# quang-ha/lammps-sph-multiphase

Measured on AMD Instinct MI355X. Metric: particle-steps/s + achieved HBM GB/s, 1M-particle taitwater+rhosum, 1/2/4/8 GPUs, higher is better.
Workload: dtype f64

## Files before the change

### include/sph_hip.h

```cpp
#ifndef SPH_HIP_H
#define SPH_HIP_H

#include <stdint.h>

#ifdef __cplusplus
extern "C" {
#endif

#define SPH_HIP_ABI_VERSION 2

#define SPH_HIP_OK 0
#define SPH_HIP_EINVAL (-1)
#define SPH_HIP_ENODEV (-2)
#define SPH_HIP_ERUNTIME (-3)
#define SPH_HIP_ENOMEM (-4)
#define SPH_HIP_ECOMM (-5)
#define SPH_HIP_EOVERFLOW (-6)

#define SPH_LIST_FULL 0
#define SPH_LIST_HALF 1

#define SPH_VISC_MONAGHAN 0
#define SPH_VISC_MORRIS 1

// ... 124 lines not shown
  int rank;
  int sort;
  int kernel_path;
  const sph_engine_mp_config *mp;
} sph_engine_config;

typedef struct {
  int64_t step;
  int nlocal, nghost;
  int64_t nbr_full;
  int nbr_builds;
  int nbr_maxrow;
  int staged;
  int stage_max;
  double ms_rhosum, ms_tait, ms_heat, ms_integrate, ms_comm, ms_neigh;
  int64_t n_rhosum, n_tait, n_heat, n_neigh;
  int blk_nbig;
  int inner_rows;
  int inner_live;
  int flags;
  int64_t inner_refresh;
} sph_engine_stats;

#define SPH_STAT_RHO_FUSED (1 << 0)
#define SPH_STAT_BLK_R32 (1 << 1)
#define SPH_STAT_BLK_BIGIMG (1 << 2)
#define SPH_STAT_BLK_NOPRE (1 << 3)
#define SPH_STAT_BLK_ROWRETRY (1 << 4)
#define SPH_STAT_BLK_IMGRETRY (1 << 5)
#define SPH_STAT_MP_W4 (1 << 6)
#define SPH_STAT_MP_POW (1 << 7)
#define SPH_STAT_MP_ROW (1 << 8)
#define SPH_STAT_MP_RHO_LISTFILL (1 << 9)

typedef struct sph_engine sph_engine;

int sph_engine_create(int device, const sph_engine_config *cfg, sph_engine **out);
int sph_engine_destroy(sph_engine *e);

int sph_engine_comm_uid(void *uid128);
int sph_engine_comm_init(sph_engine *e, const void *uid128, int nranks, int rank);
int sph_engine_comm_loopback(sph_engine *e, int on);
typedef struct sph_local_world sph_local_world;
int sph_local_world_create(int nranks, sph_local_world **out);
int sph_local_world_destroy(sph_local_world *w);
int sph_engine_comm_local(sph_engine *e, sph_local_world *w, int rank);
int sph_engine_comm_ipc(sph_engine *e, const char *name, int nranks, int rank, int mode);
#define SPH_TUNE_OVERLAP 1
#define SPH_TUNE_BLKUMF 2
int sph_engine_tune(sph_engine *e, int key, int value);
int sph_engine_set_tags(sph_engine *e, const int *tags);

int sph_engine_set_atoms(sph_engine *e, int n, const double *x, const double *v,
                         const int *type, const double *rho, const double *en,
                         const double *cv);
int sph_engine_set_atoms_multiphase(sph_engine *e, const double *rmass, const double *cv,
                                    const double *cg);
int sph_engine_phase_change(sph_engine *e, const sph_phasechange_params *p, int nevery,
                            int seed);
int sph_engine_atom_sort(sph_engine *e, int sortfreq, double binsize);

#define SPH_REGION_SPHERE 0
#define SPH_REGION_BLOCK 1
typedef struct {
  int style;
  int interior;
  double xc, yc, zc, radius;
  double xlo, xhi, ylo, yhi, zlo, zhi;
} sph_region;

#define SPH_MAX_SETMESO 8
#define SPH_SET_RHO 0
#define SPH_SET_E 1
#define SPH_SET_T 2
#define SPH_SET_DE 3
typedef struct {
  int what;
  double value;
  int type_mask;
  int region_mode;
  sph_region region;
} sph_setmeso;
int sph_engine_setmeso(sph_engine *e, const sph_setmeso *fix);
// ... 44 lines not shown
```

### lammps-sph-multiphase_amd/__init__.py

```python
from __future__ import annotations

import ctypes as C
import os

import numpy as np

HERE = os.path.dirname(os.path.abspath(__file__))
LIB_PATH = os.environ.get("SPH_HIP_LIB") or os.path.join(HERE, "libsph_hip.so")
HEADER = os.path.join(os.path.dirname(HERE), "include", "sph_hip.h")

SPH_LIST_FULL, SPH_LIST_HALF = 0, 1
SPH_VISC_MONAGHAN, SPH_VISC_MORRIS = 0, 1
SPH_MAXTYPES = 8
_NT2 = (SPH_MAXTYPES + 1) ** 2

ERRORS = {-1: "EINVAL", -2: "ENODEV", -3: "ERUNTIME", -4: "ENOMEM", -5: "ECOMM",
          -6: "EOVERFLOW"}


class HipError(RuntimeError):
    def __init__(self, code: int, msg: str):
        super().__init__(f"sph_hip {ERRORS.get(code, code)}: {msg}")
        self.code = code

# ... 151 lines not shown
    "sph_hip_host_arrays": (_i, [_vp, _i, _vp, _vp, _vp, _vp, _vp, _vp, _vp]),
    "sph_hip_list_csr": (_i, [_vp, _i, _i, _lp, _ip]),
    "sph_hip_build_list": (_i, [_vp, _i, C.c_int64, _dp]),
    "sph_hip_list_numneigh": (_i, [_vp, _ip]),
    "sph_hip_rhosum": (_i, [_vp, _dp]),
    "sph_hip_taitwater": (_i, [_vp, _dp, _dp, _dp, _vp]),
    "sph_hip_heatconduction": (_i, [_vp, _dp]),
    "sph_hip_atoms_multiphase": (_i, [_vp, _dp, _vp]),
    "sph_hip_rhosum_multiphase_coeff": (_i, [_vp, _dp]),
    "sph_hip_rhosum_multiphase": (_i, [_vp, _dp]),
    "sph_hip_taitwater_multiphase_coeff": (_i, [_vp, _dp, _dp, _dp, _dp, _dp, _dp]),
    "sph_hip_taitwater_multiphase": (_i, [_vp, _dp]),
    "sph_hip_heatconduction_phasechange_coeff": (_i, [_vp, _dp, _vp, _vp, _dp]),
    "sph_hip_heatconduction_phasechange": (_i, [_vp, _dp]),
    "sph_hip_colorgradient_coeff": (_i, [_vp, _dp, _dp]),
    "sph_hip_colorgradient": (_i, [_vp, _dp]),
    "sph_hip_set_timing": (_i, [_vp, _i]),
    "sph_hip_last_kernel_ms": (_i, [_vp, _dp]),
    "sph_hip_surfacetension_coeff": (_i, [_vp, _dp]),
    "sph_hip_surfacetension": (_i, [_vp, _dp, _dp]),
    "sph_hip_phasechange": (_i, [_vp, _vp, C.POINTER(_i), _dp, _dp, _dp, _dp, _i,
                                 C.POINTER(_i), _vp, _vp]),
    "sph_hip_phasechange_finish": (_i, [_i, _dp, _dp, _dp]),
    "sph_engine_create": (_i, [_i, C.POINTER(EngineConfig), C.POINTER(_vp)]),
    "sph_engine_destroy": (_i, [_vp]),
    "sph_engine_comm_uid": (_i, [_vp]),
    "sph_engine_comm_init": (_i, [_vp, _vp, _i, _i]),
    "sph_engine_comm_loopback": (_i, [_vp, _i]),
    "sph_local_world_create": (_i, [_i, C.POINTER(_vp)]),
    "sph_local_world_destroy": (_i, [_vp]),
    "sph_engine_comm_local": (_i, [_vp, _vp, _i]),
    "sph_engine_comm_ipc": (_i, [_vp, C.c_char_p, _i, _i, _i]),
    "sph_engine_tune": (_i, [_vp, _i, _i]),
    "sph_engine_set_tags": (_i, [_vp, _ip]),
    "sph_engine_set_atoms": (_i, [_vp, _i, _dp, _dp, _ip, _dp, _vp, _vp]),
    "sph_engine_setup": (_i, [_vp]),
    "sph_engine_run": (_i, [_vp, _i]),
    "sph_engine_nlocal": (_i, [_vp]),
    "sph_engine_get_atoms": (_i, [_vp, _vp, _vp, _vp, _vp, _vp, _vp, _vp, _vp]),
    "sph_engine_neighbor_counts": (_i, [_vp, _ip]),
    "sph_engine_stats_get": (_i, [_vp, C.POINTER(EngineStats)]),
    "sph_engine_set_timing": (_i, [_vp, _i]),
    "sph_engine_sync": (_i, [_vp]),
    "sph_engine_pair_passes": (_i, [_vp, _i]),
    "sph_engine_rebuild_passes": (_i, [_vp, _i]),
    "sph_engine_set_atoms_multiphase": (_i, [_vp, _dp, _vp, _vp]),
    "sph_engine_phase_change": (_i, [_vp, _vp, _i, _i]),
    "sph_engine_atom_sort": (_i, [_vp, _i, C.c_double]),
    "sph_engine_get_atoms_multiphase": (_i, [_vp, _vp, _vp, _vp, _vp, _vp, _vp]),
    "sph_engine_write_restart": (_i, [_vp, _vp, C.c_int64, C.POINTER(_i)]),
    "sph_engine_read_restart": (_i, [_vp, _i, _dp]),
}


def load() -> C.CDLL:
    global _lib
    if _lib is None:
        if not os.path.exists(LIB_PATH):
            raise HipError(-2, f"{LIB_PATH} not built (run `make -C lammps-sph-multiphase_amd`)")
        L = C.CDLL(LIB_PATH)
        for name, (res, args) in EXPORTS.items():
            fn = getattr(L, name)
            fn.restype = res
            fn.argtypes = args
        _lib = L
    return _lib
# ... 444 lines not shown
            for c in classes:
                mask |= 1 << c
            _chk(self.L.sph_engine_set_timing(self.h, mask << 1))
        else:
            _chk(self.L.sph_engine_set_timing(self.h, 1 if on else 0))

    @property
    def nlocal(self):
        return self.L.sph_engine_nlocal(self.h)

    def get_atoms(self):
        n = self.nlocal
        out = {k: np.zeros((n, 3)) for k in ("x", "v", "f")}
        out.update({k: np.zeros(n) for k in ("rho", "e", "drho", "de")})
        out["tag"] = np.zeros(n, dtype=np.int32)
        _chk(self.L.sph_engine_get_atoms(self.h, out["x"].ctypes.data, out["v"].ctypes.data,
                                         out["rho"].ctypes.data, out["e"].ctypes.data,
                                         out["f"].ctypes.data, out["drho"].ctypes.data,
                                         out["de"].ctypes.data, out["tag"].ctypes.data))
        return out

    def set_tags(self, tags):
        tags = np.ascontiguousarray(tags, dtype=np.int32)
        _chk(self.L.sph_engine_set_tags(self.h, tags))

    def comm_local(self, world: "LocalWorld", rank: int):
        _chk(self.L.sph_engine_comm_local(self.h, world.h, rank))
        self._world = world

    def comm_init(self, uid: bytes, nranks: int, rank: int):
        buf = C.create_string_buffer(bytes(uid), 128)
        _chk(self.L.sph_engine_comm_init(self.h, buf, nranks, rank))

    TUNE_OVERLAP, TUNE_BLKUMF = 1, 2

    def tune(self, key: int, value: int):
        _chk(self.L.sph_engine_tune(self.h, key, int(value)))

    IPC_DEVICE, IPC_HOST = 0, 1

    def comm_ipc(self, name: str, nranks: int, rank: int, mode: int = 0):
        _chk(self.L.sph_engine_comm_ipc(self.h, name.encode(), nranks, rank, int(mode)))

    def comm_loopback(self, on: bool = True):
        _chk(self.L.sph_engine_comm_loopback(self.h, 1 if on else 0))

    def neighbor_counts(self):
        c = np.zeros(self.nlocal, dtype=np.int32)
        _chk(self.L.sph_engine_neighbor_counts(self.h, c))
        return c

    STAT_RHO_FUSED, STAT_BLK_R32, STAT_BLK_BIGIMG = 1 << 0, 1 << 1, 1 << 2
    STAT_BLK_NOPRE, STAT_BLK_ROWRETRY, STAT_BLK_IMGRETRY = 1 << 3, 1 << 4, 1 << 5
    STAT_MP_W4, STAT_MP_POW, STAT_MP_ROW, STAT_MP_RHO_LISTFILL = 1 << 6, 1 << 7, 1 << 8, 1 << 9

    def stats(self) -> dict:
        s = EngineStats()
        _chk(self.L.sph_engine_stats_get(self.h, C.byref(s)))
        return s.as_dict()


def unpack_restart_records(buf):
    buf = np.asarray(buf)
    mp = buf.shape[1] == 21
    ints = (lambda c: buf[:, c].astype(np.int64)) if mp else (lambda c: buf[:, c].view(np.int64))
    img = ints(7)
    d = {"x": buf[:, 1:4], "tag": ints(4), "type": ints(5), "image": img,
         "image_xyz": np.stack([(img & 1023) - 512, ((img >> 10) & 1023) - 512,
                                ((img >> 20) & 1023) - 512], 1)}
    return d


def write_dump_custom(fp, step, atoms, columns, boxlo, boxhi, boundary="pp pp pp"):
    lo, hi = np.asarray(boxlo, float), np.asarray(boxhi, float)
    prd = hi - lo
    n = atoms["x"].shape[0]
    img = atoms.get("image", np.zeros((n, 3), np.int64))
    cols = []
    for c in columns:
        if c == "id":
            cols.append((atoms["tag"] + 1, True))
        elif c == "type":
            cols.append((atoms["type"], True))
        elif c in ("x", "y", "z"):
            cols.append((atoms["x"][:, "xyz".index(c)], False))
        elif c in ("xs", "ys", "zs"):
            k = "xyz".index(c[0])
# ... 26 lines not shown
```

### lammps-sph-multiphase_amd/csrc/sph_engine.hip

```cpp
#include <hip/hip_runtime.h>
#include <hipcub/hipcub.hpp>
#include <rocprofiler-sdk-roctx/roctx.h>

#include <algorithm>
#include <chrono>
#include <cstring>
#include <cmath>
#include <vector>

#include "sph_coef.h"
#include "sph_comm.h"
#include "sph_dispatch.h"
#include "sph_blk_kernels.h"
#include "sph_engine_kernels.h"
#include "sph_engine_mp.h"
#include "sph_fix_kernels.h"
#include "sph_ipc.h"
#include "sph_mp2_kernels.h"
#include "sph_pc.h"
#include "sph_row2_kernels.h"
#include "sph_util.h"

using namespace sph;

// ... 154 lines not shown
  bool global_tags = false;
  int last_build = 0;

  DBuf<double4> xf, vr;
  DBuf<double> en;
  DBuf<int> ty;
  DBuf<double4> vel, fo;
  DBuf<double> de;
  DBuf<int> tag;
  DBuf<double4> xf2, vr2, vel2;
  DBuf<double> en2;
  DBuf<int> ty2, tag2;
  DBuf<int> gowner, gimg;
  DBuf<int> gorank, goidx;
  bool dr_ok = false;
  std::vector<int> dr_peer;
  std::vector<size_t> dr_soff, dr_roff;
  DBuf<int> dr_sidx, dr_rslot, dr_self, dr_req;
  DBuf<int> dr_byq, dr_byg, dr_hist;
  int dr_nself = 0;
  std::vector<const void *> dr_sb;
  std::vector<void *> dr_rb;
  std::vector<size_t> dr_sbytes, dr_rbytes;
  DBuf<unsigned char> flags;
  DBuf<int> sel, nsel;
  Bins bn{};
  int nbins = 0;
  QBins qb{};
  int nqbins = 0;
  DBuf<int> qbeg, tb, xpos;
  DBuf<double4> xb;
  DBuf<unsigned> bkey, bkey2;
  DBuf<int> bidx, bidx2;
  DBuf<int> cnt, off, nbr;
  int64_t nbr_total = 0;
  int nbr_builds = 0, nbr_maxrow = 0;
  int64_t inner_refreshes = 0;
  bool strided = false;
  int list_stride = 0;
  int list_perm_g = 0;
  bool list_tbits = false;
  bool blk = false;
  int blk_sh = 0, blk_um = 0, blk_umf = 0, blk_sstride = 0, blk_rowcap = 0;
  DBuf<int> ulist, ucnt, kcnt;
  DBuf<unsigned short> snbr;
  DBuf<int> uilist, uicnt;
  bool blk_ksmall = false;
  int blk_kover = 0;
  int blk_flags = 0, blk_retry = 0;
  int mp_flags = 0;
  DBuf<unsigned short> snbi;
  DBuf<int> icnt, moved;
  DBuf<double4> x0;
  double inner_margin = 0.0;
  bool inner = false, inner_written = false;
  DBuf<int> nbs;
  DBuf<int> mx, ccnt;
  DBuf<long long> blen;
  DBuf<unsigned char> tmp;
  int *h_scalar = nullptr;
  int *h_small = nullptr;

  bool timing = false;
  int timing_mask = 0;
  struct EvPair {
    hipEvent_t a, b;
// ... 49 lines not shown
    }
    pending.clear();
  }

  void tmp_reserve(size_t b) { tmp.reserve(b); }

  void ensure_atoms(size_t nall, bool keep) {
    xf.reserve(nall, keep, s);
    vr.reserve(nall, keep, s);
    en.reserve(nall, keep, s);
    ty.reserve(nall, keep, s);
    if (mp) {
      vel.reserve(nall, keep, s);
      rm.reserve(nall, keep, s);
      cvv.reserve(nall, keep, s);
      cg.reserve(nall, keep, s);
    }
  }
  void mpx_copy(int n, const int *src, int first, DBuf<double> &buf) {
    if (!mp || n <= 0) return;
    buf.reserve((size_t)MPX * n, false, s);
    hipLaunchKernelGGL(k_mpx_pack, dim3(blocks(n)), dim3(BLK), 0, s, n, src, vel.p, rm.p, cvv.p,
                       cg.p, buf.p);
    hipLaunchKernelGGL(k_mpx_unpack, dim3(blocks(n)), dim3(BLK), 0, s, n, (const int *)nullptr,
                       first, buf.p, vel.p, rm.p, cvv.p, cg.p);
  }
  bool nt1() const { return cfg.ntypes == 1; }
  int blk_visc() const {
    if (nt1() && cfg.tait_visc == SPH_VISC_MONAGHAN && hc.tait[3].viscC == 0.0)
      return BLK_VISC_NONE;
    return cfg.tait_visc;
  }

  void sort_owned() {
    if (nlocal < 1) return;
    const int n = nlocal;
    bkey.reserve(n);
    bkey2.reserve(n);
    bidx.reserve(n);
    bidx2.reserve(n);
    const int div = morton_div();
    Bins kbn = bn;
    for (int k = 0; k < 3; k++)
      if (bn.nb[k] > 1) {
        kbn.nb[k] = bn.nb[k] * div;
        kbn.inv[k] = bn.inv[k] * div;
      }
    if (want_blk()) {
      for (int k = 0; k < 3; k++) {
        const double ext = subhi[k] - sublo[k];
        if (k >= cfg.dim || ext <= 0.0) {
          kbn.lo[k] = sublo[k];
          kbn.nb[k] = 1;
          kbn.inv[k] = 0.0;
          continue;
        }
        const int nc0 = std::max(1, (int)std::ceil(ext / (cutneighmax / div)));
        int nc = 1;
        while (nc < nc0 && nc < 1024) nc *= 2;
        if (!hil_pow2()) nc = std::min(nc0, 1024);
        kbn.lo[k] = sublo[k];
        kbn.nb[k] = nc;
        kbn.inv[k] = nc / ext;
      }
    }
    const bool mort = kbn.nb[0] <= 1024 && kbn.nb[1] <= 1024 && kbn.nb[2] <= 1024;
    if (!mort) kbn = bn;
    int cb = 1;
    const int mx3 = std::max(kbn.nb[0], std::max(kbn.nb[1], kbn.nb[2]));
    while ((1 << cb) < mx3) cb++;
    const bool hil = mort && want_blk() && cb >= 2;
    hipLaunchKernelGGL(k_bin_keys, dim3(blocks(n)), dim3(BLK), 0, s, n, 0, kbn, xf.p, bkey.p,
                       bidx.p, hil ? cb + 1 : (mort ? 1 : 0), cfg.dim);
    int kb = 1;
    if (mort) {
      kb = cb * (hil ? cfg.dim : 3);
    } else {
      while ((1u << kb) < (unsigned)nbins && kb < 32) kb++;
    }
    size_t tb = 0;
    SPH_HIP_TRY(hipcub::DeviceRadixSort::SortPairs(nullptr, tb, bkey.p, bkey2.p, bidx.p, bidx2.p, n, 0, kb, s));
    tmp_reserve(tb);
    SPH_HIP_TRY(hipcub::DeviceRadixSort::SortPairs(tmp.p, tb, bkey.p, bkey2.p, bidx.p, bidx2.p, n, 0, kb, s));
    if (mp) {
      xbuf.reserve((size_t)MPX * n, false, s);
      hipLaunchKernelGGL(k_mpx_pack, dim3(blocks(n)), dim3(BLK), 0, s, n, bidx2.p, vel.p, rm.p,
                         cvv.p, cg.p, xbuf.p);
    }
    grow_twins();
    hipLaunchKernelGGL(k_permute, dim3(blocks(n)), dim3(BLK), 0, s, n, bidx2.p, xf.p, vr.p,
                       en.p, ty.p, vel.p, tag.p, xf2.p, vr2.p, en2.p, ty2.p, vel2.p, tag2.p);
    std::swap(xf, xf2);
    std::swap(vr, vr2);
    std::swap(en, en2);
    std::swap(ty, ty2);
    std::swap(vel, vel2);
    std::swap(tag, tag2);
    if (pc) {
      lidx2.reserve_exact(lidx.cap);
      hipLaunchKernelGGL(k_lidx_take, dim3(blocks(n)), dim3(BLK), 0, s, n, bidx2.p, lidx.p, 0,
                         (const int *)nullptr, lidx2.p);
      std::swap(lidx, lidx2);
    }
    if (mp)
      hipLaunchKernelGGL(k_mpx_unpack, dim3(blocks(n)), dim3(BLK), 0, s, n, (const int *)nullptr,
                         0, xbuf.p, vel.p, rm.p, cvv.p, cg.p);
  }

  void grow_twins() {
    xf2.reserve_exact(xf.cap);
    vr2.reserve_exact(vr.cap);
    en2.reserve_exact(en.cap);
    ty2.reserve_exact(ty.cap);
    vel2.reserve_exact(vel.cap);
    tag2.reserve_exact(tag.cap);
  }
// ... 718 lines not shown
      const double ext = bn.nb[k] > 0 && bn.inv[k] > 0.0 ? bn.nb[k] / bn.inv[k] : 0.0;
      int nb = 1;
      if (k < cfg.dim) {
        nb = (int)(ext / (0.5 * cutneighmax / (k == 0 ? fx : 1)));
        if (nb < 1) nb = 1;
        if (nb > 8192) nb = 8192;
      }
      qb.lo[k] = bn.lo[k];
      qb.nb[k] = nb;
      qb.inv[k] = (k < cfg.dim) ? nb / ext : 0.0;
      qb.size[k] = (k < cfg.dim) ? ext / nb : 1.0;
    }
    qb.cutmaxsq = cutneighmax * cutneighmax;
    nqbins = qb.nb[0] * qb.nb[1] * qb.nb[2];
  }

  void bin_q() {
    const int nall = nlocal + nghost;
    Bins b;
    for (int k = 0; k < 3; k++) {
      b.lo[k] = qb.lo[k];
      b.inv[k] = qb.inv[k];
      b.nb[k] = qb.nb[k];
    }
    bkey.reserve(nall);
    bkey2.reserve(nall);
    bidx.reserve(nall);
    bidx2.reserve(nall);
    qbeg.reserve(nqbins + 1);
    xb.reserve(nall);
    tb.reserve(nall);
    SPH_REQUIRE(!mp || (long long)nall < MP_MAXALL, SPH_HIP_EOVERFLOW,
                "multiphase lists index at most 2^28 atoms per rank (%d)", nall);
    hipLaunchKernelGGL(k_bin_keys, dim3(blocks(nall)), dim3(BLK), 0, s, nall, 0, b, xf.p,
                       bkey.p, bidx.p, 0);
    int endbit = 1;
    while ((1u << endbit) < (unsigned)nqbins && endbit < 32) endbit++;
    size_t tbytes = 0;
    SPH_HIP_TRY(hipcub::DeviceRadixSort::SortPairs(nullptr, tbytes, bkey.p, bkey2.p, bidx.p, bidx2.p, nall, 0, endbit, s));
    tmp_reserve(tbytes);
    SPH_HIP_TRY(hipcub::DeviceRadixSort::SortPairs(tmp.p, tbytes, bkey.p, bkey2.p, bidx.p, bidx2.p, nall, 0, endbit, s));
    hipLaunchKernelGGL(k_lower_bound, dim3(blocks(nqbins + 1)), dim3(BLK), 0, s, nqbins, nall,
                       0, bkey2.p, qbeg.p);
    xpos.reserve(nall);
    hipLaunchKernelGGL(k_bin_copy, dim3(blocks(nall)), dim3(BLK), 0, s, nall, bidx2.p, xf.p,
                       ty.p, xb.p, tb.p, xpos.p, mp ? 1 : 0);
  }
  void list_q(bool csr, const double4 *xi = nullptr) {
    const int n = nlocal, nall = nlocal + nghost;
    const double4 *const xi_src = xi ? xi : xf.p;
    const bool rho = mp && !xi && rhofuse_env() && mpc.rhosum_nstep > 0 &&
                     step % mpc.rhosum_nstep == 0;
    SPH_REQUIRE(!mp || (long long)nall < MP_MAXALL, SPH_HIP_EOVERFLOW,
                "multiphase lists index at most 2^28 atoms per rank (%d)", nall);
    if (rho) rho_tmp.reserve(nlocal + nghost);
    rho_fused_step = rho ? step : -1;
    ccnt.reserve(n + 1);
    off.reserve(n + 1);
    constexpr int G = 8;
    dim3 grid(grid_for_rows(n, G)), block(BLK);
    auto launch = [&](bool fill, int stride, int *dst = nullptr) {
      if (n == 0) return;
      const bool t = nt1();
      const int *const tgp = (mp && !mp2_symmetric(hm)) ? tag.p : (const int *)nullptr;
      int *const cnt_out = (!fill || stride > 0) ? ccnt.p : (int *)nullptr;
      int *const rows = dst ? dst : nbr.p;
// ... 1097 lines not shown
                                                   : cfg->boxlo[k] + e->box.prd[k] * hi;
      auto at = [&](int dx, int dy, int dz) {
        const int l[3] = {(e->myloc[0] + dx + e->pg[0]) % e->pg[0],
                          (e->myloc[1] + dy + e->pg[1]) % e->pg[1],
                          (e->myloc[2] + dz + e->pg[2]) % e->pg[2]};
        return (l[2] * e->pg[1] + l[1]) * e->pg[0] + l[0];
      };
      e->procneigh[k][0] = at(k == 0 ? -1 : 0, k == 1 ? -1 : 0, k == 2 ? -1 : 0);
      e->procneigh[k][1] = at(k == 0 ? 1 : 0, k == 1 ? 1 : 0, k == 2 ? 1 : 0);
      if (e->box.periodic[k])
        SPH_REQUIRE(e->cutghost < e->box.prd[k], SPH_HIP_EINVAL,
                    "ghost cutoff %g >= box length %g in dim %d (multi-hop borders unsupported)",
                    e->cutghost, e->box.prd[k], k);
      if (e->pg[k] > 1)
        SPH_REQUIRE(e->cutghost < e->subhi[k] - e->sublo[k], SPH_HIP_EINVAL,
                    "ghost cutoff %g >= brick width %g in dim %d (multi-hop swaps unsupported)",
                    e->cutghost, e->subhi[k] - e->sublo[k], k);
    }
    e->sc.dtv = cfg->dt;
    e->sc.dtf = 0.5 * cfg->dt * (cfg->ftm2v > 0 ? cfg->ftm2v : 1.0);
    for (int t = 0; t <= nt; t++) e->sc.mass[t] = cfg->mass[t];
    e->sc.stationary_mask = cfg->stationary_mask;
    e->setup_bins_geometry();
    SPH_HIP_TRY(hipStreamCreateWithFlags(&e->s, hipStreamNonBlocking));
    SPH_HIP_TRY(hipMalloc(&e->dc, sizeof(Coefs)));
    SPH_HIP_TRY(hipMemcpy(e->dc, &e->hc, sizeof(Coefs), hipMemcpyHostToDevice));
    if (e->mp) {
      SPH_HIP_TRY(hipMalloc(&e->dm, sizeof(MpCoefs)));
      mp_inverses(e->hm);
      SPH_HIP_TRY(hipMemcpy(e->dm, &e->hm, sizeof(MpCoefs), hipMemcpyHostToDevice));
    }
    SPH_HIP_TRY(hipHostMalloc(&e->h_scalar, sizeof(int)));
    SPH_HIP_TRY(hipHostMalloc(&e->h_small, 16 * sizeof(int)));
  } catch (...) {
    delete e;
    throw;
  }
  e->overlap = false;
  *out = e;
  SPH_API_END
}

int sph_engine_destroy(sph_engine *e) {
  if (!e) return SPH_HIP_OK;
  (void)hipSetDevice(e->device);
  if (e->s) (void)hipStreamSynchronize(e->s);
  if (e->s2) (void)hipStreamSynchronize(e->s2);
  for (auto *b : {&e->xf, &e->vr, &e->vel, &e->fo, &e->xf2, &e->vr2, &e->vel2, &e->xb}) b->release();
  for (auto *b : {&e->en, &e->en2, &e->de, &e->rm, &e->cvv, &e->rho_tmp, &e->dmass, &e->xbuf,
                  &e->xbuf2})
    b->release();
  for (auto *b : {&e->rhoS, &e->rhoF}) b->release();
  for (auto *b : {&e->cg, &e->cgS, &e->cgF, &e->recA, &e->recK, &e->recF, &e->recS}) b->release();
  if (e->dm) (void)hipFree(e->dm);
  for (auto *b : {&e->nbs, &e->gorank, &e->goidx, &e->dr_sidx, &e->dr_rslot, &e->dr_self, &e->dr_req, &e->dr_byq, &e->dr_byg, &e->dr_hist, &e->pc_flag,
                  &e->pc_cand, &e->pc_otag, &e->pc_idx})
    b->release();
  for (auto *b : {&e->pc_rec, &e->pc_gat, &e->pc_Wd, &e->pc_vals, &e->pc_nrec, &e->pc_v0,
                  &e->pc_v1})
    b->release();
  e->pc_k0.release();
  e->pc_k1.release();
  e->pc_cnt.release();
  e->red_part.release();
  e->red_out.release();
  for (auto *b : {&e->ty, &e->ty2, &e->tag, &e->tag2, &e->gowner, &e->gimg, &e->sel, &e->nsel,
                  &e->bidx, &e->bidx2, &e->cnt, &e->off, &e->nbr, &e->mx,
                  &e->ccnt, &e->qbeg, &e->tb, &e->xpos, &e->sel2, &e->rows_in, &e->rows_bd,
                  &e->ulist, &e->ucnt, &e->kcnt, &e->uilist, &e->uicnt})
    b->release();
  for (auto *b : {&e->bkey, &e->bkey2}) b->release();
  for (auto *b : {&e->flags, &e->tmp, &e->cbs, &e->cbr, &e->flag2, &e->fl_in, &e->fl_bd}) b->release();
  e->snbr.release();
  e->snbi.release();
  e->icnt.release();
  e->moved.release();
  e->x0.release();
  e->blen.release();
  for (auto &sw : e->swaps) sw.list.release();
  for (auto &p : e->pending) {
    (void)hipEventDestroy(p.a);
    (void)hipEventDestroy(p.b);
  }
  for (auto ev : e->evpool) (void)hipEventDestroy(ev);
  if (e->h_scalar) (void)hipHostFree(e->h_scalar);
  if (e->h_small) (void)hipHostFree(e->h_small);
  delete e->tr;
  if (e->dc) (void)hipFree(e->dc);
  if (e->ev_fork) (void)hipEventDestroy(e->ev_fork);
  if (e->ev_join) (void)hipEventDestroy(e->ev_join);
  if (e->s2) (void)hipStreamDestroy(e->s2);
  if (e->s) (void)hipStreamDestroy(e->s);
  delete e;
  return SPH_HIP_OK;
}

int sph_engine_set_atoms(sph_engine *e, int n, const double *x, const double *v,
                         const int *type, const double *rho, const double *en,
                         const double *cv) {
  SPH_API_BEGIN
  SPH_REQUIRE(e && n >= 0 && (n == 0 || (x && v && type && rho)), SPH_HIP_EINVAL,
              "sph_engine_set_atoms: bad argument");
  SPH_HIP_TRY(hipSetDevice(e->device));
  for (int i = 0; i < n; i++)
// ... 473 lines not shown
  st->nghost = e->nghost;
  st->nbr_full = e->list_entries();
  st->nbr_builds = e->nbr_builds;
  st->nbr_maxrow = e->nbr_maxrow;
  st->staged = e->blk ? 1 : 0;
  st->stage_max = e->blk ? e->blk_um : 0;
  st->ms_rhosum = e->ms[T_RHO];
  st->ms_tait = e->ms[T_TAIT];
  st->ms_heat = e->ms[T_HEAT];
  st->ms_integrate = e->ms[T_INT];
  st->ms_comm = e->ms[T_COMM];
  st->ms_neigh = e->ms[T_NEIGH];
  st->n_rhosum = e->nlaunch[T_RHO];
  st->n_tait = e->nlaunch[T_TAIT];
  st->n_heat = e->nlaunch[T_HEAT];
  st->n_neigh = e->nlaunch[T_NEIGH];
  st->blk_nbig = 0;
  if (e->blk && e->mx.p) {
    SPH_HIP_TRY(hipMemcpyAsync(&st->blk_nbig, e->mx.p + 9, sizeof(int), hipMemcpyDeviceToHost,
                               e->s));
    SPH_HIP_TRY(hipStreamSynchronize(e->s));
  }
  st->inner_rows = e->inner ? 1 : 0;
  st->inner_live = 0;
  if (e->inner && e->moved.p) {
    int mv = 1;
    SPH_HIP_TRY(hipMemcpyAsync(&mv, e->moved_flag(), sizeof(int), hipMemcpyDeviceToHost, e->s));
    SPH_HIP_TRY(hipStreamSynchronize(e->s));
    st->inner_live = mv == 0 ? 1 : 0;
  }
  st->flags = (e->rho_fused_step >= 0 && e->rho_fused_step == e->step) ? SPH_STAT_RHO_FUSED : 0;
  if (e->blk) st->flags |= e->blk_flags;
  if (e->mp) st->flags |= e->mp_flags;
  st->inner_refresh = e->inner_refreshes;
  SPH_API_END
}

int sph_engine_set_timing(sph_engine *e, int on) {
  SPH_API_BEGIN
  SPH_REQUIRE(e, SPH_HIP_EINVAL, "sph_engine_set_timing: NULL engine");
  SPH_HIP_TRY(hipSetDevice(e->device));
  e->harvest();
  e->timing_mask = on == 1 ? (1 << T_NCLASS) - 1 : (on > 1 ? (on >> 1) & ((1 << T_NCLASS) - 1) : 0);
  e->timing = e->timing_mask != 0;
  for (int k = 0; k < T_NCLASS; k++) {
    e->ms[k] = 0.0;
    e->nlaunch[k] = 0;
  }
  SPH_API_END
}

int sph_engine_sync(sph_engine *e) {
  SPH_API_BEGIN
  SPH_REQUIRE(e, SPH_HIP_EINVAL, "sph_engine_sync: NULL engine");
  SPH_HIP_TRY(hipSetDevice(e->device));
  SPH_HIP_TRY(hipStreamSynchronize(e->s));
  SPH_API_END
}

int sph_engine_comm_uid(void *uid128) {
  SPH_API_BEGIN
  SPH_REQUIRE(uid128, SPH_HIP_EINVAL, "sph_engine_comm_uid: NULL buffer");
  static_assert(sizeof(ncclUniqueId) == 128, "ncclUniqueId is 128 bytes");
  ncclUniqueId id;
  SPH_NCCL_TRY(ncclGetUniqueId(&id));
  memcpy(uid128, &id, sizeof(id));
// ... 41 lines not shown

int sph_local_world_destroy(sph_local_world *w) {
  delete reinterpret_cast<LocalWorld *>(w);
  return SPH_HIP_OK;
}

int sph_engine_comm_local(sph_engine *e, sph_local_world *w, int rank) {
  SPH_API_BEGIN
  SPH_REQUIRE(e && w, SPH_HIP_EINVAL, "sph_engine_comm_local: NULL argument");
  LocalWorld *lw = reinterpret_cast<LocalWorld *>(w);
  SPH_REQUIRE(rank >= 0 && rank < lw->n, SPH_HIP_EINVAL, "rank %d outside [0,%d)", rank, lw->n);
  attach(e, new LocalTransport(lw, rank));
  SPH_API_END
}

int sph_engine_comm_ipc(sph_engine *e, const char *name, int nranks, int rank, int mode) {
  SPH_API_BEGIN
  SPH_REQUIRE(e && name, SPH_HIP_EINVAL, "sph_engine_comm_ipc: NULL argument");
  SPH_HIP_TRY(hipSetDevice(e->device));
  attach(e, new IpcTransport(name, nranks, rank, mode, e->device));
  SPH_API_END
}

int sph_engine_tune(sph_engine *e, int key, int value) {
  SPH_API_BEGIN
  SPH_REQUIRE(e, SPH_HIP_EINVAL, "sph_engine_tune: NULL engine");
  SPH_REQUIRE(!e->setup_done, SPH_HIP_EINVAL, "sph_engine_tune: before sph_engine_setup");
  switch (key) {
    case SPH_TUNE_OVERLAP: e->overlap = value != 0; break;
    case SPH_TUNE_BLKUMF:
      SPH_REQUIRE(value >= 0, SPH_HIP_EINVAL, "sph_engine_tune: BLKUMF %d < 0", value);
      e->blkumf = value;
      break;
    default: SPH_REQUIRE(false, SPH_HIP_EINVAL, "sph_engine_tune: unknown key %d", key);
  }
  SPH_API_END
}

int sph_engine_set_tags(sph_engine *e, const int *tags) {
  SPH_API_BEGIN
  SPH_REQUIRE(e && (tags || e->nlocal == 0), SPH_HIP_EINVAL, "sph_engine_set_tags: bad argument");
  SPH_HIP_TRY(hipSetDevice(e->device));
  int mx = -1;
  for (int i = 0; i < e->nlocal; i++) {
    SPH_REQUIRE(tags[i] >= 0 && tags[i] < (1 << 30), SPH_HIP_EINVAL,
                "sph_engine_set_tags: tag %d outside [0, 2^30)", tags[i]);
    mx = std::max(mx, tags[i]);
  }
  if (e->nlocal)
    SPH_HIP_TRY(hipMemcpy(e->tag.p, tags, e->nlocal * sizeof(int), hipMemcpyHostToDevice));
  e->global_tags = true;
  e->tag_next = mx + 1;
  e->pc_tags_agreed = false;
  e->lidx_valid = false;
  SPH_API_END
}

int sph_engine_atom_sort(sph_engine *e, int sortfreq, double binsize) {
  SPH_API_BEGIN
  SPH_REQUIRE(e, SPH_HIP_EINVAL, "sph_engine_atom_sort: NULL engine");
  SPH_REQUIRE(sortfreq >= 0 && binsize >= 0.0, SPH_HIP_EINVAL, "Illegal atom_modify command");
  e->sortfreq = sortfreq;
  e->sort_binsize = binsize;
  SPH_API_END
}

}
```

### lammps-sph-multiphase_amd/csrc/sph_engine_kernels.h

```cpp
#pragma once
#include <hip/hip_runtime.h>

#include "sph_kernels.h"
#include "sph_mp2_kernels.h"

namespace sph {

struct StepConst {
  double dtv, dtf;
  double mass[MAXT + 1];
  int stationary_mask;
  const double4 *x0;
  double lim2;
  int *moved;
};

__device__ __forceinline__ void inner_check(const StepConst &sc, int i, const double4 &x) {
  if (!sc.x0) return;
  const double4 a = sc.x0[i];
  const double dx = x.x - a.x, dy = x.y - a.y, dz = x.z - a.z;
  if (dx * dx + dy * dy + dz * dz > sc.lim2) atomicOr(sc.moved, 1);
}

static __global__ void k_inner_ghosts(int ng, int nlocal, StepConst sc,
// ... 483 lines not shown
                                 double4 *__restrict__ xf2, double4 *__restrict__ vr2,
                                 double *__restrict__ en2, int *__restrict__ ty2,
                                 double4 *__restrict__ vel2, int *__restrict__ tag2) {
  const int i = blockIdx.x * blockDim.x + threadIdx.x;
  if (i >= n) return;
  const int s = perm[i];
  xf2[i] = xf[s];
  vr2[i] = vr[s];
  en2[i] = en[s];
  ty2[i] = ty[s];
  vel2[i] = vel[s];
  tag2[i] = tag[s];
}

struct QBins {
  double lo[3], inv[3], size[3];
  int nb[3];
  double cutmaxsq;
};

static __global__ void k_bin_copy(int n, const int *__restrict__ perm,
                                  const double4 *__restrict__ xf, const int *__restrict__ ty,
                                  double4 *__restrict__ xb, int *__restrict__ tb,
                                  int *__restrict__ xpos = nullptr, int tpack = 0) {
  const int p = blockIdx.x * blockDim.x + threadIdx.x;
  if (p >= n) return;
  const int j = perm[p];
  const double4 x = xf[j];
  xb[p] = make_double4(x.x, x.y, x.z, (double)(tpack ? j | ((ty[j] - 1) << 28) : j));
  tb[p] = ty[j];
  if (xpos) xpos[j] = p;
}

__device__ __forceinline__ double slab_gap(double v, int b, int c, double lo, double size) {
  if (b == c) return 0.0;
  const double edge = (b < c) ? lo + (b + 1) * size : lo + b * size;
  const double g = (b < c) ? v - edge : edge - v;
  return fmax(g - 1e-6 * size, 0.0);
}

__device__ __forceinline__ bool half_keep(int i, int j, int nlocal, const double4 &xi,
                                          const double4 &xj) {
  if (j < nlocal) return i < j;
  if (xj.z < xi.z) return false;
  if (xj.z == xi.z) {
    if (xj.y < xi.y) return false;
    if (xj.y == xi.y && xj.x < xi.x) return false;
  }
  return true;
}

template <int G, int U, bool FILL, bool NT1, bool RHO = false, bool TP = false>
__global__ void __launch_bounds__(256)
k_neigh3(int nlocal, QBins q, int dim, const double4 *__restrict__ xf,
         const int *__restrict__ ty, const double4 *__restrict__ xb,
         const int *__restrict__ tb, const int *__restrict__ beg,
         const Coefs *__restrict__ cf, int *__restrict__ cnt, const int *__restrict__ off,
         int *__restrict__ nbr, int stride, int *__restrict__ ovf, int perm_g, int tbits,
         const MpCoefs *__restrict__ mc = nullptr,
         const double *__restrict__ rm = nullptr, double *__restrict__ rho = nullptr,
         const int *__restrict__ tg = nullptr) {
  constexpr int R = 2, NB = (2 * R + 1) * (2 * R + 1), GR = 256 / G, KB = (NB + G - 1) / G;
  static_assert(!RHO || FILL, "the rhosum terms ride on the fill passes");
  __shared__ double s_cns[NT2];
  __shared__ double s_rcs[RHO ? NT2 : 1], s_rih[RHO ? NT2 : 1], s_rwn[RHO ? NT2 : 1];
  __shared__ double s_hr[RHO ? GR : 1][RHO ? G * U : 1];
// ... 232 lines not shown
```

Measured before the change: 1.840 billion.

## Replace radix sort with counting sort for neighbor binning and atom sort

```diff
diff --git a/include/sph_hip.h b/include/sph_hip.h
--- a/include/sph_hip.h
+++ b/include/sph_hip.h
@@ -180,6 +180,8 @@
 #define SPH_STAT_MP_POW (1 << 7)
 #define SPH_STAT_MP_ROW (1 << 8)
 #define SPH_STAT_MP_RHO_LISTFILL (1 << 9)
+#define SPH_STAT_CSORT_BINS (1 << 10)
+#define SPH_STAT_CSORT_ROWS (1 << 11)
 
 typedef struct sph_engine sph_engine;
 
@@ -196,7 +198,9 @@
 int sph_engine_comm_ipc(sph_engine *e, const char *name, int nranks, int rank, int mode);
 #define SPH_TUNE_OVERLAP 1
 #define SPH_TUNE_BLKUMF 2
+#define SPH_TUNE_CSORT 3
 int sph_engine_tune(sph_engine *e, int key, int value);
+int sph_engine_csort_paths(sph_engine *e, int *mask);
 int sph_engine_set_tags(sph_engine *e, const int *tags);
 
 int sph_engine_set_atoms(sph_engine *e, int n, const double *x, const double *v,
diff --git a/lammps-sph-multiphase_amd/__init__.py b/lammps-sph-multiphase_amd/__init__.py
--- a/lammps-sph-multiphase_amd/__init__.py
+++ b/lammps-sph-multiphase_amd/__init__.py
@@ -207,6 +207,7 @@
     "sph_engine_comm_local": (_i, [_vp, _vp, _i]),
     "sph_engine_comm_ipc": (_i, [_vp, C.c_char_p, _i, _i, _i]),
     "sph_engine_tune": (_i, [_vp, _i, _i]),
+    "sph_engine_csort_paths": (_i, [_vp, C.POINTER(_i)]),
     "sph_engine_set_tags": (_i, [_vp, _ip]),
     "sph_engine_set_atoms": (_i, [_vp, _i, _dp, _dp, _ip, _dp, _vp, _vp]),
     "sph_engine_setup": (_i, [_vp]),
@@ -717,7 +718,7 @@
         buf = C.create_string_buffer(bytes(uid), 128)
         _chk(self.L.sph_engine_comm_init(self.h, buf, nranks, rank))
 
-    TUNE_OVERLAP, TUNE_BLKUMF = 1, 2
+    TUNE_OVERLAP, TUNE_BLKUMF, TUNE_CSORT = 1, 2, 3
 
     def tune(self, key: int, value: int):
         _chk(self.L.sph_engine_tune(self.h, key, int(value)))
@@ -738,6 +739,12 @@
     STAT_RHO_FUSED, STAT_BLK_R32, STAT_BLK_BIGIMG = 1 << 0, 1 << 1, 1 << 2
     STAT_BLK_NOPRE, STAT_BLK_ROWRETRY, STAT_BLK_IMGRETRY = 1 << 3, 1 << 4, 1 << 5
     STAT_MP_W4, STAT_MP_POW, STAT_MP_ROW, STAT_MP_RHO_LISTFILL = 1 << 6, 1 << 7, 1 << 8, 1 << 9
+    STAT_CSORT_BINS, STAT_CSORT_ROWS = 1 << 10, 1 << 11
+
+    def csort_paths(self) -> int:
+        m = _i(0)
+        _chk(self.L.sph_engine_csort_paths(self.h, C.byref(m)))
+        return m.value
 
     def stats(self) -> dict:
         s = EngineStats()
diff --git a/lammps-sph-multiphase_amd/csrc/sph_engine.hip b/lammps-sph-multiphase_amd/csrc/sph_engine.hip
--- a/lammps-sph-multiphase_amd/csrc/sph_engine.hip
+++ b/lammps-sph-multiphase_amd/csrc/sph_engine.hip
@@ -210,6 +210,13 @@
   DBuf<double4> xb;
   DBuf<unsigned> bkey, bkey2;
   DBuf<int> bidx, bidx2;
+  DBuf<int> cs_cnt, cs_beg, cs_mx;
+  int *h_cs = nullptr;
+  hipEvent_t cs_ev[2] = {nullptr, nullptr};
+  bool cs_pending[2] = {false, false};
+  int cs_prev[2] = {-1, -1};
+  int csort = 1;
+  int cs_flags = 0;
   DBuf<int> cnt, off, nbr;
   int64_t nbr_total = 0;
   int nbr_builds = 0, nbr_maxrow = 0;
@@ -325,6 +332,43 @@
     return cfg.tait_visc;
   }
 
+  static constexpr int CS_KFLOOR = 1 << 16, CS_KPERN = 4, CS_KMAX = 1 << 24;
+  bool cs_count(int w, int n, long long K0, const Bins &b, int morton, int hdim,
+                DBuf<int> &begb) {
+    if (!csort || n < 1 || K0 < 1 || K0 > CS_KMAX) return false;
+    if (K0 > CS_KFLOOR && K0 > (long long)CS_KPERN * n) return false;
+    const int K = (int)K0;
+    begb.reserve((size_t)K + 1);
+    int *const beg = begb.p;
+    int prev = cs_prev[w];
+    if (cs_pending[w]) {
+      SPH_HIP_TRY(hipEventSynchronize(cs_ev[w]));
+      cs_pending[w] = false;
+      prev = h_cs[w];
+    }
+    if (!setup_done) prev = -1;
+    cs_cnt.reserve((size_t)K + 1);
+    cs_mx.reserve(2);
+    SPH_HIP_TRY(hipMemsetAsync(cs_cnt.p, 0, ((size_t)K + 1) * sizeof(int), s));
+    SPH_HIP_TRY(hipMemsetAsync(cs_mx.p + w, 0, sizeof(int), s));
+    hipLaunchKernelGGL(k_cs_hist, dim3(blocks(n)), dim3(BLK), 0, s, n, b, xf.p, bkey.p,
+                       (int *)bkey2.p, cs_cnt.p, K, cs_mx.p + w, morton, hdim);
+    SPH_HIP_TRY(hipMemcpyAsync(h_cs + w, cs_mx.p + w, sizeof(int), hipMemcpyDeviceToHost, s));
+    if (prev != 0) {
+      SPH_HIP_TRY(hipStreamSynchronize(s));
+      cs_prev[w] = h_cs[w];
+      if (cs_prev[w] > CS_CAP) return false;
+    } else {
+      SPH_HIP_TRY(hipEventRecord(cs_ev[w], s));
+      cs_pending[w] = true;
+    }
+    size_t tb = 0;
+    SPH_HIP_TRY(hipcub::DeviceScan::ExclusiveSum(nullptr, tb, cs_cnt.p, beg, K + 1, s));
+    tmp_reserve(tb);
+    SPH_HIP_TRY(hipcub::DeviceScan::ExclusiveSum(tmp.p, tb, cs_cnt.p, beg, K + 1, s));
+    return true;
+  }
+
   void sort_owned() {
     if (nlocal < 1) return;
     const int n = nlocal;
@@ -363,18 +407,30 @@
     const int mx3 = std::max(kbn.nb[0], std::max(kbn.nb[1], kbn.nb[2]));
     while ((1 << cb) < mx3) cb++;
     const bool hil = mort && want_blk() && cb >= 2;
-    hipLaunchKernelGGL(k_bin_keys, dim3(blocks(n)), dim3(BLK), 0, s, n, 0, kbn, xf.p, bkey.p,
-                       bidx.p, hil ? cb + 1 : (mort ? 1 : 0), cfg.dim);
+    const int morton = hil ? cb + 1 : (mort ? 1 : 0);
     int kb = 1;
     if (mort) {
       kb = cb * (hil ? cfg.dim : 3);
     } else {
       while ((1u << kb) < (unsigned)nbins && kb < 32) kb++;
     }
-    size_t tb = 0;
-    SPH_HIP_TRY(hipcub::DeviceRadixSort::SortPairs(nullptr, tb, bkey.p, bkey2.p, bidx.p, bidx2.p, n, 0, kb, s));
-    tmp_reserve(tb);
-    SPH_HIP_TRY(hipcub::DeviceRadixSort::SortPairs(tmp.p, tb, bkey.p, bkey2.p, bidx.p, bidx2.p, n, 0, kb, s));
+    cs_flags &= ~SPH_STAT_CSORT_ROWS;
+    if (cs_count(1, n, 1ll << kb, kbn, morton, cfg.dim, cs_beg)) {
+      hipLaunchKernelGGL(k_cs_scatter, dim3(blocks(n)), dim3(BLK), 0, s, n, bkey.p,
+                         (const int *)bkey2.p, cs_beg.p, bidx.p);
+      hipLaunchKernelGGL(k_cs_place<false>, dim3(blocks(n)), dim3(BLK), 0, s, n, bkey.p,
+                         cs_beg.p, bidx.p, bidx2.p, (const double4 *)nullptr,
+                         (const int *)nullptr, (double4 *)nullptr, (int *)nullptr,
+                         (int *)nullptr, 0);
+      cs_flags |= SPH_STAT_CSORT_ROWS;
+    } else {
+      hipLaunchKernelGGL(k_bin_keys, dim3(blocks(n)), dim3(BLK), 0, s, n, 0, kbn, xf.p, bkey.p,
+                         bidx.p, morton, cfg.dim);
+      size_t tb = 0;
+      SPH_HIP_TRY(hipcub::DeviceRadixSort::SortPairs(nullptr, tb, bkey.p, bkey2.p, bidx.p, bidx2.p, n, 0, kb, s));
+      tmp_reserve(tb);
+      SPH_HIP_TRY(hipcub::DeviceRadixSort::SortPairs(tmp.p, tb, bkey.p, bkey2.p, bidx.p, bidx2.p, n, 0, kb, s));
+    }
     if (mp) {
       xbuf.reserve((size_t)MPX * n, false, s);
       hipLaunchKernelGGL(k_mpx_pack, dim3(blocks(n)), dim3(BLK), 0, s, n, bidx2.p, vel.p, rm.p,
@@ -1159,6 +1215,26 @@
     tb.reserve(nall);
     SPH_REQUIRE(!mp || (long long)nall < MP_MAXALL, SPH_HIP_EOVERFLOW,
                 "multiphase lists index at most 2^28 atoms per rank (%d)", nall);
+    xpos.reserve(nall);
+    cs_flags &= ~SPH_STAT_CSORT_BINS;
+    if (cs_count(0, nall, nqbins, b, 0, 3, qbeg)) {
+      hipLaunchKernelGGL(k_cs_scatter, dim3(blocks(nall)), dim3(BLK), 0, s, nall, bkey.p,
+                         (const int *)bkey2.p, qbeg.p, bidx.p);
+      if (csort == 2) {
+        hipLaunchKernelGGL(k_cs_place<false>, dim3(blocks(nall)), dim3(BLK), 0, s, nall, bkey.p,
+                           qbeg.p, bidx.p, bidx2.p, (const double4 *)nullptr,
+                           (const int *)nullptr, (double4 *)nullptr, (int *)nullptr,
+                           (int *)nullptr, 0);
+        hipLaunchKernelGGL(k_bin_copy, dim3(blocks(nall)), dim3(BLK), 0, s, nall, bidx2.p, xf.p,
+                           ty.p, xb.p, tb.p, xpos.p, mp ? 1 : 0);
+      } else {
+        hipLaunchKernelGGL(k_cs_place<true>, dim3(blocks(nall)), dim3(BLK), 0, s, nall, bkey.p,
+                           qbeg.p, bidx.p, (int *)nullptr, xf.p, ty.p, xb.p, tb.p, xpos.p,
+                           mp ? 1 : 0);
+      }
+      cs_flags |= SPH_STAT_CSORT_BINS;
+      return;
+    }
     hipLaunchKernelGGL(k_bin_keys, dim3(blocks(nall)), dim3(BLK), 0, s, nall, 0, b, xf.p,
                        bkey.p, bidx.p, 0);
     int endbit = 1;
@@ -2322,6 +2398,8 @@
     }
     SPH_HIP_TRY(hipHostMalloc(&e->h_scalar, sizeof(int)));
     SPH_HIP_TRY(hipHostMalloc(&e->h_small, 16 * sizeof(int)));
+    SPH_HIP_TRY(hipHostMalloc(&e->h_cs, 2 * sizeof(int)));
+    for (auto &ev : e->cs_ev) SPH_HIP_TRY(hipEventCreateWithFlags(&ev, hipEventDisableTiming));
   } catch (...) {
     delete e;
     throw;
@@ -2360,6 +2438,10 @@
                   &e->ulist, &e->ucnt, &e->kcnt, &e->uilist, &e->uicnt})
     b->release();
   for (auto *b : {&e->bkey, &e->bkey2}) b->release();
+  for (auto *b : {&e->cs_cnt, &e->cs_beg, &e->cs_mx}) b->release();
+  for (auto ev : e->cs_ev)
+    if (ev) (void)hipEventDestroy(ev);
+  if (e->h_cs) (void)hipHostFree(e->h_cs);
   for (auto *b : {&e->flags, &e->tmp, &e->cbs, &e->cbr, &e->flag2, &e->fl_in, &e->fl_bd}) b->release();
   e->snbr.release();
   e->snbi.release();
@@ -2899,6 +2981,7 @@
   st->flags = (e->rho_fused_step >= 0 && e->rho_fused_step == e->step) ? SPH_STAT_RHO_FUSED : 0;
   if (e->blk) st->flags |= e->blk_flags;
   if (e->mp) st->flags |= e->mp_flags;
+  if (e->blk || e->mp) st->flags |= e->cs_flags;
   st->inner_refresh = e->inner_refreshes;
   SPH_API_END
 }
@@ -3006,8 +3089,19 @@
       SPH_REQUIRE(value >= 0, SPH_HIP_EINVAL, "sph_engine_tune: BLKUMF %d < 0", value);
       e->blkumf = value;
       break;
+    case SPH_TUNE_CSORT:
+      SPH_REQUIRE(value >= 0 && value <= 2, SPH_HIP_EINVAL, "sph_engine_tune: CSORT %d", value);
+      e->csort = value;
+      break;
     default: SPH_REQUIRE(false, SPH_HIP_EINVAL, "sph_engine_tune: unknown key %d", key);
   }
+  SPH_API_END
+}
+
+int sph_engine_csort_paths(sph_engine *e, int *mask) {
+  SPH_API_BEGIN
+  SPH_REQUIRE(e && mask, SPH_HIP_EINVAL, "sph_engine_csort_paths: NULL argument");
+  *mask = e->cs_flags;
   SPH_API_END
 }
 
diff --git a/lammps-sph-multiphase_amd/csrc/sph_engine_kernels.h b/lammps-sph-multiphase_amd/csrc/sph_engine_kernels.h
--- a/lammps-sph-multiphase_amd/csrc/sph_engine_kernels.h
+++ b/lammps-sph-multiphase_amd/csrc/sph_engine_kernels.h
@@ -539,6 +539,63 @@
   if (xpos) xpos[j] = p;
 }
 
+#define CS_CAP 64
+
+static __global__ void k_cs_hist(int n, Bins bn, const double4 *__restrict__ xf,
+                                 unsigned *__restrict__ key, int *__restrict__ slot,
+                                 int *__restrict__ cnt, int K, int *__restrict__ mx, int morton,
+                                 int hdim) {
+  const int k = blockIdx.x * blockDim.x + threadIdx.x;
+  if (k >= n) return;
+  const double4 x = xf[k];
+  const int cx = bin_coord(x.x, bn.lo[0], bn.inv[0], bn.nb[0]);
+  const int cy = bin_coord(x.y, bn.lo[1], bn.inv[1], bn.nb[1]);
+  const int cz = bin_coord(x.z, bn.lo[2], bn.inv[2], bn.nb[2]);
+  unsigned q;
+  if (morton > 1)
+    q = hilbert_key(hdim, (unsigned)cx, (unsigned)cy, (unsigned)cz, morton - 1);
+  else
+    q = morton ? (spread3(cx) | (spread3(cy) << 1) | (spread3(cz) << 2))
+               : (unsigned)((cz * bn.nb[1] + cy) * bn.nb[0] + cx);
+  if (q >= (unsigned)K) q = (unsigned)K - 1;
+  key[k] = q;
+  const int c = atomicAdd(&cnt[q], 1);
+  slot[k] = c;
+  if (c + 1 > CS_CAP / 2) atomicMax(mx, c + 1);
+}
+
+static __global__ void k_cs_scatter(int n, const unsigned *__restrict__ key,
+                                    const int *__restrict__ slot, const int *__restrict__ beg,
+                                    int *__restrict__ list) {
+  const int k = blockIdx.x * blockDim.x + threadIdx.x;
+  if (k >= n) return;
+  list[beg[key[k]] + slot[k]] = k;
+}
+
+template <bool COPY>
+__global__ void __launch_bounds__(256)
+k_cs_place(int n, const unsigned *__restrict__ key, const int *__restrict__ beg,
+           const int *__restrict__ list, int *__restrict__ perm,
+           const double4 *__restrict__ xf, const int *__restrict__ ty,
+           double4 *__restrict__ xb, int *__restrict__ tb, int *__restrict__ xpos, int tpack) {
+  const int k = blockIdx.x * blockDim.x + threadIdx.x;
+  if (k >= n) return;
+  const unsigned q = key[k];
+  const int st = beg[q], en = beg[q + 1];
+  int r = 0;
+  for (int p = st; p < en; p++) r += list[p] < k ? 1 : 0;
+  const int p = st + r;
+  if (COPY) {
+    const double4 x = xf[k];
+    const int t = ty[k];
+    xb[p] = make_double4(x.x, x.y, x.z, (double)(tpack ? k | ((t - 1) << 28) : k));
+    tb[p] = t;
+    xpos[k] = p;
+  } else {
+    perm[p] = k;
+  }
+}
+
 __device__ __forceinline__ double slab_gap(double v, int b, int c, double lo, double size) {
   if (b == c) return 0.0;
   const double edge = (b < c) ? lo + (b + 1) * size : lo + b * size;
```

New measurement: 1.899 billion (median of 6 runs). 3.2% higher.
